# hanruihua/RDA-planner

Measured on AMD Instinct MI355X. Metric: MPC steps/sec (ADMM early stop or iter_num cap: see residuals), T=20, N_obs=200, higher is better.
Workload: dtype f64; 1 GPU; north-star: acker rectangle robot, T=20, N_obs=200 static seeded polygons, E=4, iter_num=4, iter_threshold=0.2, ro1=200; parallelism=single GPU

## Files before the change

rda_planner_amd/csrc/lammuz_device.h:

```cpp
#pragma once
#include <hip/hip_runtime.h>
#include <math.h>

#pragma clang fp contract(on)

namespace lmz {

constexpr int EMAX = 8;
constexpr int RMAX = 8;
constexpr double SIGN_TOL = 1e-12;

struct WaveLDS {
    double A[EMAX][2];
    double b[EMAX];
    double q[EMAX];
    double M[EMAX][2];
    unsigned char lamc[40];
    double vtx[28][2];
    int npv, nlv;
};
struct RobotLDS {
    double G[RMAX][2];
    double h[RMAX];
    unsigned char muc[40]; int nmv;
    double rv[28][2]; int nrv;
};

struct Sol {
    double cost; int id;
    double m, H0, H1;
    int i1, i2, j1, j2;
    double l1, l2, g1, g2;
};

struct MuCand { int k; int j0, j1; double gx, gy, eta; double P00, P01, P10, P11, det, r0, r1, rr;
                double iden;
                double idet; };

__device__ __forceinline__ void gamma_star(const MuCand &mc, double chi, double ro2, double delta,
                                           double t, double e0, double e1,
                                           double &ga0, double &ga1, double &m, double &H0, double &H1)
{
    if (mc.k == 0) { m = t; H0 = e0; H1 = e1; ga0 = 0; ga1 = 0; return; }
    if (mc.k == 1) {
        double ga = (chi * mc.eta * t - delta * mc.eta - ro2 * (mc.gx * e0 + mc.gy * e1)) * mc.iden;
        ga0 = ga; ga1 = 0; m = t - mc.eta * ga; H0 = e0 + ga * mc.gx; H1 = e1 + ga * mc.gy;
        return;
    }
    double re = mc.r0 * e0 + mc.r1 * e1;
    double beta = (delta - chi * (t + re)) * mc.iden;
    H0 = -beta * mc.r0; H1 = -beta * mc.r1;
    double d0 = H0 - e0, d1 = H1 - e1;
    ga0 = (mc.P11 * d0 - mc.P01 * d1) * mc.idet;
    ga1 = (-mc.P10 * d0 + mc.P00 * d1) * mc.idet;
    m = t + re + beta * mc.rr;
}

__device__ __forceinline__ int trs2(double q11, double q12, double q22, double c0, double c1, bool disc,
                                    double &x0, double &x1, double &x2, double &x3)
{
// ... 267 lines not shown
{
    if (lane < P.E) {
        double ax = W.A[lane][0], ay = W.A[lane][1];
        W.q[lane] = ax * P.px + ay * P.py - W.b[lane];
        W.M[lane][0] = ax * P.cs + ay * P.sn;
        W.M[lane][1] = -ax * P.sn + ay * P.cs;
    }
}

__device__ __forceinline__ void build_lists(WaveLDS &W, int E, int norm2, int lane)
{
    if (norm2) {
        if (lane == 0) { W.lamc[0] = 1; W.lamc[1] = 2; W.lamc[2] = 0; W.npv = 0; W.nlv = 3; }
    } else {
        bool vp = false; double vx = 0, vy = 0;
        if (lane < E * (E - 1) / 2) {
            int i1, i2; decode_pair(lane, E, i1, i2);
            const double a00 = W.A[i1][0], a01 = W.A[i1][1], a10 = W.A[i2][0], a11 = W.A[i2][1];
            const double det = a00 * a11 - a01 * a10;
            if (det != 0 && det * det > 1e-24 * (a00 * a00 + a01 * a01) * (a10 * a10 + a11 * a11)) {
                const double wx = W.b[i1] * a11 - a01 * W.b[i2], wy = a00 * W.b[i2] - W.b[i1] * a10, sg = det > 0 ? 1.0 : -1.0, ad = fabs(det);
                vp = true;
                for (int k = 0; k < E; ++k) {
                    const double ak0 = W.A[k][0], ak1 = W.A[k][1], bk = W.b[k];
                    const double viol = sg * (ak0 * wx + ak1 * wy - bk * det);
                    if (viol > 1e-9 * (ad + fabs(bk) * ad + fabs(ak0 * wx) + fabs(ak1 * wy))) vp = false;
                }
                vx = wx / det; vy = wy / det;
            }
        }
        const bool vs = lane < E && (W.A[lane < E ? lane : 0][0] != 0 || W.A[lane < E ? lane : 0][1] != 0);
        const unsigned long long bp = __ballot(vp), bs = __ballot(vs), below = (1ull << lane) - 1;
        const int npv = __popcll(bp), nsv = __popcll(bs);
        if (vp) { const int k = __popcll(bp & below); W.lamc[k] = (unsigned char)(1 + E + lane); W.vtx[k][0] = vx; W.vtx[k][1] = vy; }
        if (vs) W.lamc[npv + __popcll(bs & below)] = (unsigned char)(1 + lane);
        if (lane == 0) { W.lamc[npv + nsv] = 0; W.npv = npv; W.nlv = npv + nsv + 1; }
    }
}

__device__ __forceinline__ void wave_sync()
{
    __builtin_amdgcn_fence(__ATOMIC_RELEASE, "workgroup");
    __builtin_amdgcn_wave_barrier();
    __builtin_amdgcn_fence(__ATOMIC_ACQUIRE, "workgroup");
}

__device__ __forceinline__ void prepare_wave(WaveLDS &W, const Params &P, int lane)
{
    pose_products(W, P, lane);
    build_lists(W, P.E, P.norm2, lane);
    wave_sync();
}

__device__ __forceinline__ void solve_wave(WaveLDS &W, const RobotLDS &Rb, const Params &P, int lane, Sol &best)
{
    const int nm = 1 + P.R + P.R * (P.R - 1) / 2;
    const int nlv = W.nlv, nmv = Rb.nmv;
    const int half = nlv * nmv;
    best.cost = INFINITY; best.id = 0x7fffffff;
    best.m = 0; best.H0 = 0; best.H1 = 0; best.i1 = best.i2 = best.j1 = best.j2 = -1;
    best.l1 = best.l2 = best.g1 = best.g2 = 0;
    long long tprev = P.prof ? clock64() : 0;
    auto mark = [&](int k) { if (P.prof && lane == 0) { long long now = clock64(); P.prof[k] += now - tprev; tprev = now; } };
    for (int ic = 0; ic < 2; ++ic) {
        int itn = 0;
        for (int c = lane; c < half; c += 64) {
            const int ilx = c / nmv, il = W.lamc[ilx], im = Rb.muc[c - ilx * nmv];
            Sol s;
            if (eval_candidate(W, Rb, P, il, im, ic, s)) {
                s.id = 2 * (il * nm + im) + ic;
                if (s.cost < best.cost || (s.cost == best.cost && s.id < best.id)) best = s;
            }
            mark(1 + 2 * ic + (itn < 1 ? itn : 1)); ++itn;
        }
        double bc = best.cost; int bid = best.id;
#pragma unroll
        for (int off = 32; off >= 1; off >>= 1) {
            double oc = __shfl_xor(bc, off, 64); int oid = __shfl_xor(bid, off, 64);
            if (oc < bc || (oc == bc && oid < bid)) { bc = oc; bid = oid; }
        }
        unsigned long long win = __ballot(best.id == bid);
        int src = __ffsll((long long)win) - 1;
        best.cost = __shfl(best.cost, src, 64); best.id = bid;
        best.m = __shfl(best.m, src, 64); best.H0 = __shfl(best.H0, src, 64); best.H1 = __shfl(best.H1, src, 64);
        best.i1 = __shfl(best.i1, src, 64); best.i2 = __shfl(best.i2, src, 64);
        best.j1 = __shfl(best.j1, src, 64); best.j2 = __shfl(best.j2, src, 64);
        best.l1 = __shfl(best.l1, src, 64); best.l2 = __shfl(best.l2, src, 64);
        best.g1 = __shfl(best.g1, src, 64); best.g2 = __shfl(best.g2, src, 64);
        mark(5 + ic);
        if (best.m >= 0) break;
        if (ic == 0) best.cost += 0.5 * best.m * best.m;
    }
}

template <int CTRL> __device__ __forceinline__ double dpp_mov_f64(double v)
{
    int lo = __builtin_amdgcn_update_dpp(0, __double2loint(v), CTRL, 0xf, 0xf, false);
    int hi = __builtin_amdgcn_update_dpp(0, __double2hiint(v), CTRL, 0xf, 0xf, false);
    return __hiloint2double(hi, lo);
}
__device__ __forceinline__ double wave_max(double v)
{
    double o;
    o = dpp_mov_f64<0xB1>(v); v = o > v ? o : v;
    o = dpp_mov_f64<0x4E>(v); v = o > v ? o : v;
    o = dpp_mov_f64<0x141>(v); v = o > v ? o : v;
    o = dpp_mov_f64<0x140>(v); v = o > v ? o : v;
    o = __shfl_xor(v, 16, 64); v = o > v ? o : v;
    o = __shfl_xor(v, 32, 64); v = o > v ? o : v;
    return v;
}

__device__ __forceinline__ double row_max(double v)
{
    double o;
    o = dpp_mov_f64<0xB1>(v); v = o > v ? o : v;
    o = dpp_mov_f64<0x4E>(v); v = o > v ? o : v;
    o = dpp_mov_f64<0x141>(v); v = o > v ? o : v;
    o = dpp_mov_f64<0x140>(v); v = o > v ? o : v;
    return v;
}
template <int GW> struct Grp {
    static __device__ __forceinline__ unsigned long long ballot(bool p, int lane)
    {
        const unsigned long long b = __ballot(p);
        if (GW == 64) return b;
        return (b >> (lane & 48)) & 0xffffull;
    }
    static __device__ __forceinline__ double max(double v) { return GW == 64 ? wave_max(v) : row_max(v); }
    template <typename Tv> static __device__ __forceinline__ Tv bcast(Tv v, int src) { return __shfl(v, src, GW); }
};

__device__ __forceinline__ int support_neighbour(int c, int n, const unsigned char *cand, int ncand, int k)
{
    if (c == 0) { int seen = 0; for (int q = 0; q < ncand; ++q) { const int v = cand[q]; if (v >= 1 && v <= n) { if (seen == k) return v; ++seen; } } return -1; }
    if (c <= n) {
        if (k == 0) return 0;
        int seen = 1;
        for (int q = 0; q < ncand; ++q) {
            const int v = cand[q];
            if (v > n) { int a, b; decode_pair(v - 1 - n, n, a, b); if (a == c - 1 || b == c - 1) { if (seen == k) return v; ++seen; } }
        }
// ... 225 lines not shown
    if (isinf(tlo)) { chl = 0; shl = 1; } else { const double r = rsqrt(1.0 + tlo * tlo); chl = r; shl = tlo * r; }
    const double Cr = chh * chl + shh * shl, Sr = shh * chl - chh * shl;
    const double a0 = u0 * Cr - u1 * Sr, a1 = u1 * Cr + u0 * Sr;
    int i1 = -1, i2 = -1; double l1 = 0, l2 = 0;
    if (P.norm2) { i1 = 0; i2 = 1; l1 = a0; l2 = a1; }
    else {
        const double val = lane < nv ? a0 * W.vtx[lane < nv ? lane : 0][0] + a1 * W.vtx[lane < nv ? lane : 0][1] : -INFINITY, mx = Grp<GW>::max(val);
        const int kb = __ffsll((long long)Grp<GW>::ballot(val == mx, wlane)) - 1;
        decode_pair((int)W.lamc[kb] - 1 - P.E, P.E, i1, i2);
        const double a00 = W.A[i1][0], a01 = W.A[i1][1], a10 = W.A[i2][0], a11 = W.A[i2][1], det = a00 * a11 - a01 * a10;
        l1 = (a0 * a11 - a10 * a1) / det;
        l2 = (a00 * a1 - a0 * a01) / det;
        if (l1 < -1e-9 || l2 < -1e-9) return false;
        if (l1 < 0) l1 = 0;
        if (l2 < 0) l2 = 0;
    }
    const double gx = -(P.cs * a0 + P.sn * a1) - P.xi0, gy = -(-P.sn * a0 + P.cs * a1) - P.xi1;
    int j1, j2; double g1, g2;
    {
        const double val = lane < nr ? gx * Rb.rv[lane < nr ? lane : 0][0] + gy * Rb.rv[lane < nr ? lane : 0][1] : -INFINITY, mx = Grp<GW>::max(val);
        const int jb = __ffsll((long long)Grp<GW>::ballot(val == mx, wlane)) - 1;
        decode_pair((int)Rb.muc[jb] - 1 - P.R, P.R, j1, j2);
        const double a00 = Rb.G[j1][0], a01 = Rb.G[j1][1], a10 = Rb.G[j2][0], a11 = Rb.G[j2][1], det = a00 * a11 - a01 * a10;
        g1 = (gx * a11 - a10 * gy) / det;
        g2 = (a00 * gy - gx * a01) / det;
        if (g1 < -1e-9 || g2 < -1e-9) return false;
        if (g1 < 0) g1 = 0;
        if (g2 < 0) g2 = 0;
    }
    double m = P.kappa0 - g1 * Rb.h[j1] - g2 * Rb.h[j2];
    double H0 = P.xi0 + g1 * Rb.G[j1][0] + g2 * Rb.G[j2][0], H1 = P.xi1 + g1 * Rb.G[j1][1] + g2 * Rb.G[j2][1];
    if (P.norm2) {
        m += l1 * W.q[0] + l2 * W.q[1] - W.q[2];
        H0 += l1 * W.M[0][0] + l2 * W.M[1][0] - W.M[2][0]; H1 += l1 * W.M[0][1] + l2 * W.M[1][1] - W.M[2][1];
    } else {
        m += l1 * W.q[i1] + l2 * W.q[i2];
        H0 += l1 * W.M[i1][0] + l2 * W.M[i2][0]; H1 += l1 * W.M[i1][1] + l2 * W.M[i2][1];
    }
    if (m < 0) return false;
    best.i1 = i1; best.i2 = i2; best.l1 = l1; best.l2 = l2; best.j1 = j1; best.j2 = j2; best.g1 = g1; best.g2 = g2;
    best.m = m; best.H0 = H0; best.H1 = H1;
    return true;
}

__device__ __forceinline__ double lam_of(const Sol &s, int norm2, int e)
{
    if (norm2) {
        if (s.i1 < 0) return 0.0;
        return e == 0 ? s.l1 : (e == 1 ? s.l2 : (e == 2 ? -hypot(s.l1, s.l2) : 0.0));
    }
    return e == s.i1 ? s.l1 : (e == s.i2 ? s.l2 : 0.0);
}
__device__ __forceinline__ double mu_of(const Sol &s, int j) { return j == s.j1 ? s.g1 : (j == s.j2 ? s.g2 : 0.0); }

}

#pragma clang fp contract(fast)
```

rda_planner_amd/csrc/rda_hip.hip:

```cpp
#include <hip/hip_runtime.h>
#include <climits>
#include <cstdio>
#include <cstdlib>
#include <cstring>
#include <vector>
#include <chrono>
#include <memory>
#include <dlfcn.h>
#include "../../include/rda_hip.h"
#include "host_buf.h"
#include "lammuz_device.h"
#include "lammuz_cp_device.h"
#include "lammuz_ip_device.h"
#include "su_device.h"
#include "scene_device.h"
#include "lidar_device.h"
#include "track_device.h"
#include "rollout_device.h"

#define HIPCHK(x) do { hipError_t e_ = (x); if (e_ != hipSuccess) { \
    fprintf(stderr, "librda_hip: %s failed: %s (%s:%d)\n", #x, hipGetErrorString(e_), __FILE__, __LINE__); return RDA_ERR_HIP; } } while (0)

struct Ctrl {
    int stop, iters, su_status, ipm_iters, st_tmp, it_tmp;
// ... 467 lines not shown
    if (d.centre) lmz::central_normal_wave<64>(W, rb, P, lane, best);
    bad = bad || !(isfinite(best.cost) && isfinite(best.m) && isfinite(best.H0) && isfinite(best.H1));
    const int k = t * d.Nloc + nl;
    if (bad) {
        if (lane == 0) {
            store_row(d, k, failed_row(d, k));
            hint_write(d, hpar, n, t, -1);
            atomicAdd(&d.ctrl->lmz_fail, 1);
        }
        return;
    }
    const double znew = (d.c.accelerated ? 0.5 : 1.0) * (best.m > 0 ? best.m : 0.0);
    double res = 0;
    if (lane < E) {
        double v = lmz::lam_of(best, P.norm2, lane);
        res = (v - prev) * (v - prev); d.lam[o * E + lane] = v;
    } else if (lane < E + R) {
        int j = lane - E;
        double v = lmz::mu_of(best, j);
        res = (v - prev) * (v - prev); d.mu[o * R + j] = v;
    } else if (lane == E + R) {
        double old = d.z[zi];
        res = (znew - old) * (znew - old); d.z[zi] = znew;
    }
#pragma unroll
    for (int off = 32; off >= 1; off >>= 1) res += __shfl_xor(res, off, 64);
    if (lane == 0) {
        double ax = 0, ay = 0, bl = 0, mh = 0, gx = 0, gy = 0;
        for (int i = 0; i < E; ++i) {
            double v = lmz::lam_of(best, P.norm2, i);
            ax += v * W.A[i][0]; ay += v * W.A[i][1]; bl += v * W.b[i];
        }
        for (int j = 0; j < R; ++j) {
            double v = lmz::mu_of(best, j);
            mh += v * rb.h[j]; gx += v * rb.G[j][0]; gy += v * rb.G[j][1];
        }
        const double hx = gx + P.cs * ax + P.sn * ay, hy = gy - P.sn * ax + P.cs * ay;
        const double xin0 = P.xi0 + hx, xin1 = P.xi1 + hy;
        d.xi[2 * o] = xin0; d.xi[2 * o + 1] = xin1;
        const double im = ax * P.px + ay * P.py - bl - mh;
        const double zetan = zeta + im - dbar - znew;
        d.zeta[zi] = zetan;
        RowOut ro; ro.ax = ax; ro.ay = ay; ro.bl = bl; ro.c3 = mh + znew - zetan; ro.c4 = gx + xin0; ro.c5 = gy + xin1;
        ro.res = res; ro.hh = hx * hx + hy * hy;
        store_row(d, k, ro);
    }
}

__global__ __launch_bounds__(256) void k_lammuz(Dev d, int it) { lammuz_body(d, blockIdx.x, it); }

#ifdef RDA_LMZ_CLK
__device__ unsigned long long *g_lmz_clk = nullptr;
__device__ int *g_lmz_faillog = nullptr;
#endif
template <int MODE = 0, bool CW = false> __device__ __forceinline__ void lammuz_body_rows(const Dev &d, const int block, const int nblocks, const int it, const Fin &fin)
{
#pragma clang fp contract(on)
    constexpr int WPB = GS / 4;
    __shared__ lmz::WaveLDS wl[GS];
    __shared__ lmz::RobotLDS rb;
    __shared__ double rowv[MODE == 0 ? GS : 1][6];
    const int T = d.c.T, E = d.c.E, R = d.c.R;
#ifdef RDA_LMZ_CLK
    long long clk_prev = clock64(); const long long clk_in = clk_prev; bool clk_enum = false; const unsigned long long clk_wall_in = (unsigned long long)wall_clock64();
    unsigned long long *const clk_slot = g_lmz_clk ? g_lmz_clk + 16 * (size_t)(block * (GS / 4) + (threadIdx.x >> 6)) : nullptr;
#define LMZ_CLK(k) do { if (MODE == 0) { const long long now_ = clock64(); if (clk_slot && (threadIdx.x & 63) == 0) clk_slot[k] += (unsigned long long)(now_ - clk_prev); clk_prev = now_; } } while (0)
#else
#define LMZ_CLK(k) do { } while (0)
#endif
    int tb = 0, jb = 0;
    if (MODE != 2) { block_of(d, block, tb, jb); if (tb < 0) return; }
    const int lane = threadIdx.x & 63, wv = threadIdx.x >> 6, row = lane >> 4, gl = lane & 15;
    struct Early { double px, py, cs, sn, xi0, xi1, zeta, dbar, prev, vtx[4], A, b, G, h, zold; int cone, src, hpar, hint, npv, nlv; unsigned char lamc[3]; } ey;
    if (MODE == 0) {
        const int nl0 = jb * GS + wv * 4 + row, nl = nl0 < d.Nlive ? nl0 : 0, n = d.rank * d.Nloc + nl;
        ey.src = (d.slot_src && n < d.src_used) ? d.slot_src[n] : -1;
        ey.hpar = d.ctrl->hint_par & 1;
    }
    if (d.ctrl->stop) return;
    if (MODE == 2 && block * WPB >= d.ctrl->wl_count + (d.ctrl->wlc_count + 3) / 4) return;
    LMZ_CLK(0);
    if (MODE == 0) {
        const int t = tb, nl0 = jb * GS + wv * 4 + row, nl = nl0 < d.Nlive ? nl0 : 0, n = d.rank * d.Nloc + nl;
        const double *ps = d.pose + 4 * t;
        const size_t o = drow(d, n, t + 1), zi = drow(d, n, t), oc = (size_t)n * d.nt + (d.nt > 1 ? t + 1 : 0);
        ey.px = ps[0]; ey.py = ps[1]; ey.cs = ps[2]; ey.sn = ps[3];
        ey.xi0 = d.xi[2 * o]; ey.xi1 = d.xi[2 * o + 1]; ey.zeta = d.zeta[zi]; ey.dbar = d.dis[t]; ey.cone = d.cone[n];
        ey.zold = d.z[zi];
        ey.prev = *(gl < E ? &d.lam[o * E + gl] : (gl < E + R ? &d.mu[o * R + gl - E] : &d.lam[o * E]));
        {
            const size_t ao = ((size_t)n * d.nt + (d.nt > 1 ? t + 1 : 0)) * E;
            ey.A = d.A[ao * 2 + (gl < 2 * E ? gl : 0)]; ey.b = d.b[ao + (gl < E ? gl : 0)];
            ey.G = d.G[(int)threadIdx.x < 2 * R ? threadIdx.x : 0]; ey.h = d.h[(int)threadIdx.x < R ? threadIdx.x : 0];
        }
#pragma unroll
        for (int k = 0; k < 3; ++k) ey.lamc[k] = gl + 16 * k < d.oc_ls ? d.oc_lamc[oc * d.oc_ls + gl + 16 * k] : (unsigned char)0;
#pragma unroll
        for (int k = 0; k < 4; ++k) ey.vtx[k] = gl + 16 * k < d.oc_vs ? d.oc_vtx[oc * d.oc_vs + gl + 16 * k] : 0.0;
        ey.npv = d.oc_cnt[2 * oc]; ey.nlv = d.oc_cnt[2 * oc + 1];
        {
            const int key = (ey.src >= 0 && ey.src < d.src_cap) ? d.c.N + ey.src : n, tr = (it == 0 && t + 1 < T) ? t + 1 : t;
            ey.hint = d.hint[(size_t)(ey.hpar ^ 1) * d.hint_len + (size_t)tr * d.hint_stride + key];
        }
    }
    if (MODE == 0) {
        if ((int)threadIdx.x < 2 * R) rb.G[threadIdx.x >> 1][threadIdx.x & 1] = ey.G;
        if ((int)threadIdx.x < R) rb.h[threadIdx.x] = ey.h;
    } else {
        for (int i = threadIdx.x; i < 2 * R; i += 64 * WPB) rb.G[i >> 1][i & 1] = d.G[i];
        for (int i = threadIdx.x; i < R; i += 64 * WPB) rb.h[i] = d.h[i];
    }
    for (int i = threadIdx.x; i < 40; i += 64 * WPB) rb.muc[i] = d.muc[i];
    for (int i = threadIdx.x; i < 56; i += 64 * WPB) (&rb.rv[0][0])[i] = (&d.rv[0][0])[i];
    if (threadIdx.x == 0) { rb.nmv = d.nmv; rb.nrv = d.nrv; }
    const int cntP = MODE == 2 ? d.ctrl->wl_count : 1, cntC = MODE == 2 ? d.ctrl->wlc_count : 0;
    const int cnt = cntP + (cntC + 3) / 4;
    for (int base = MODE == 2 ? block * WPB : 0; base < cnt; base += MODE == 2 ? nblocks * WPB : 1) {
    if (MODE == 2) __syncthreads();
    const bool entry = MODE == 2 && base + wv < cnt;
// ... 63 lines not shown
    lmz::wave_sync();
    LMZ_CLK(2);
    const int hpar = MODE == 0 ? ey.hpar : (d.ctrl->hint_par & 1);
    const int hint_in = MODE == 0 ? ey.hint : (MODE != 2 ? hint_read(d, hpar, n, t, it == 0) : ((P.norm2 && live) ? hint_read(d, hpar, n, t, it == 0) : -1));
    bool ok = MODE != 2 && d.warm && lmz::solve_wave_warm<16>(W, rb, P, lane, hint_in, best);
    if (CW && MODE == 0 && d.warm && P.norm2 && live && !bad) ok = lmz::warm_circle<16>(W, rb, P, lane, hint_in, best);
    if (MODE == 2 && d.warm && P.norm2 && live && !bad) ok = lmz::warm_circle<16>(W, rb, P, lane, hint_in, best);
    LMZ_CLK(3);
    if (MODE != 2 && !live && !ok) {
        best.cost = 0; best.id = 0; best.m = -1; best.H0 = best.H1 = 0; best.i1 = best.i2 = best.j1 = best.j2 = -1;
        best.l1 = best.l2 = best.g1 = best.g2 = 0;
        ok = true;
    }
    unsigned long long need = __ballot(!ok);
    if (MODE == 2) {
        need = __ballot(live && !ok);
        if (!live) {
            best.cost = 0; best.id = 0; best.m = -1; best.H0 = best.H1 = 0; best.i1 = best.i2 = best.j1 = best.j2 = -1;
            best.l1 = best.l2 = best.g1 = best.g2 = 0;
        }
    }
#ifdef RDA_LMZ_STATS
    if (lane == 0) {
        const int nf = __popcll(need) >> 4;
        if (block == 0 && wv == 0) atomicAdd(&d.ctrl->lmz_stat[0], 1u);
        atomicAdd(&d.ctrl->lmz_stat[1], (unsigned)nf); atomicAdd(&d.ctrl->lmz_stat[2 + nf], 1u);
    }
#endif
    bool defer = false;
    if (MODE == 1) {
        defer = ((need >> (16 * row)) & 1) != 0 && !bad;
        if ((need >> (16 * row)) & 1) {
            best.cost = 0; best.id = 0; best.m = -1; best.H0 = best.H1 = 0; best.i1 = best.i2 = best.j1 = best.j2 = -1;
            best.l1 = best.l2 = best.g1 = best.g2 = 0;
        }
        if (defer && gl == 0 && live) {
            if (P.norm2) d.wl[d.wl_cap - 1 - atomicAdd(&d.ctrl->wlc_count, 1)] = t * GS * d.J + nl;
            else d.wl[atomicAdd(&d.ctrl->wl_count, 1)] = t * GS * d.J + nl;
        }
        need = 0;
    }
    if (MODE == 0) {
        struct Prm { int norm2; double px, py, cs, sn, xi0, xi1, kappa0; };
        __shared__ int nfail; __shared__ unsigned char flist[GS]; __shared__ Prm prm[GS]; __shared__ lmz::Sol sol[GS];
        if (threadIdx.x == 0) nfail = 0;
        __syncthreads();
        const bool mine = ((need >> (16 * row)) & 1) != 0;
        if (mine && gl == 0) {
            const int rid = wv * 4 + row; flist[atomicAdd(&nfail, 1)] = (unsigned char)rid;
            Prm &q = prm[rid]; q.norm2 = P.norm2; q.px = P.px; q.py = P.py; q.cs = P.cs; q.sn = P.sn; q.xi0 = P.xi0; q.xi1 = P.xi1; q.kappa0 = P.kappa0;
        }
        __syncthreads();
        const int nf = nfail;
        for (int i = wv; i < nf; i += WPB) {
            const int rid = flist[i];
            lmz::Params Pg;
            { const Prm &q = prm[rid]; Pg.E = E; Pg.R = R; Pg.norm2 = q.norm2; Pg.px = q.px; Pg.py = q.py; Pg.cs = q.cs; Pg.sn = q.sn; Pg.xi0 = q.xi0; Pg.xi1 = q.xi1;
              Pg.kappa0 = q.kappa0; Pg.ro2 = P.ro2; Pg.delta = P.delta; }
            lmz::Sol bg;
            lmz::solve_wave(wl[rid], rb, Pg, lane, bg);
            if (lane == 0) sol[rid] = bg;
        }
        __syncthreads();
        if (mine) best = sol[wv * 4 + row];
        need = 0;
#ifdef RDA_LMZ_CLK
        clk_enum = nf > 0;
        if (mine && gl == 0 && live && g_lmz_faillog) {
            const int k = atomicAdd(&g_lmz_faillog[0], 1);
            if (k < 200000) { g_lmz_faillog[1 + 3 * k] = hint_in; g_lmz_faillog[2 + 3 * k] = best.id >> 1; g_lmz_faillog[3 + 3 * k] = P.norm2; }
        }
#endif
    }
    LMZ_CLK(4);
    while (need) {
        const int g = (__ffsll((long long)need) - 1) >> 4;
        need &= ~(0xffffull << (16 * g));
        lmz::Params Pg;
        const int src = 16 * g;
        Pg.E = E; Pg.R = R; Pg.norm2 = __shfl(P.norm2, src, 64);
        Pg.px = __shfl(P.px, src, 64); Pg.py = __shfl(P.py, src, 64); Pg.cs = __shfl(P.cs, src, 64); Pg.sn = __shfl(P.sn, src, 64);
        Pg.xi0 = __shfl(P.xi0, src, 64); Pg.xi1 = __shfl(P.xi1, src, 64); Pg.kappa0 = __shfl(P.kappa0, src, 64);
        Pg.ro2 = P.ro2; Pg.delta = P.delta;
        lmz::Sol bg;
        lmz::solve_wave(wl[wv * 4 + g], rb, Pg, lane, bg);
        if (row == g) best = bg;
    }
    if (gl == 0 && live && !defer) hint_write(d, hpar, n, t, best.id >> 1);
    if (d.centre) lmz::central_normal_wave<16>(W, rb, P, lane, best);
    LMZ_CLK(5);
    bad = bad || !(isfinite(best.cost) && isfinite(best.m) && isfinite(best.H0) && isfinite(best.H1));
    const double znew = (d.c.accelerated ? 0.5 : 1.0) * (best.m > 0 ? best.m : 0.0);
    double res = 0;
    const bool wr = live && !bad && !defer;
    if (gl < E) {
        double v = lmz::lam_of(best, P.norm2, gl);
        res = (v - prev) * (v - prev); if (wr) d.lam[o * E + gl] = v;
    } else if (gl < E + R) {
        int j = gl - E;
        double v = lmz::mu_of(best, j);
        res = (v - prev) * (v - prev); if (wr) d.mu[o * R + j] = v;
    } else if (gl == E + R) {
        const double old = MODE == 0 ? ey.zold : d.z[zi];
        res = (znew - old) * (znew - old); if (wr) d.z[zi] = znew;
    }
#pragma unroll
    for (int off = 8; off >= 1; off >>= 1) res += __shfl_xor(res, off, 16);
    if (gl == 0) {
        const int k = t * d.Nloc + nl;
        RowOut ro;
        bool have = false;
        if (live && bad) {
            ro = failed_row(d, k); have = true;
            store_row(d, k, ro);
            hint_write(d, hpar, n, t, -1);
            atomicAdd(&d.ctrl->lmz_fail, 1);
        } else if (wr) {
            double ax = 0, ay = 0, bl = 0, mh = 0, gx = 0, gy = 0;
            for (int i = 0; i < E; ++i) {
                double v = lmz::lam_of(best, P.norm2, i);
                ax += v * W.A[i][0]; ay += v * W.A[i][1]; bl += v * W.b[i];
            }
            for (int j = 0; j < R; ++j) {
                double v = lmz::mu_of(best, j);
                mh += v * rb.h[j]; gx += v * rb.G[j][0]; gy += v * rb.G[j][1];
            }
            const double hx = gx + P.cs * ax + P.sn * ay, hy = gy - P.sn * ax + P.cs * ay;
            const double xin0 = P.xi0 + hx, xin1 = P.xi1 + hy;
            d.xi[2 * o] = xin0; d.xi[2 * o + 1] = xin1;
            const double im = ax * P.px + ay * P.py - bl - mh;
            const double zetan = zeta + im - dbar - znew;
            d.zeta[zi] = zetan;
            ro.ax = ax; ro.ay = ay; ro.bl = bl; ro.c3 = mh + znew - zetan; ro.c4 = gx + xin0; ro.c5 = gy + xin1;
            ro.res = res; ro.hh = hx * hx + hy * hy; have = true;
            store_row(d, k, ro);
        }
        if (MODE == 0) {
            double *rv = rowv[wv * 4 + row];
            if (have) row_record(rv, d, ro, px0, py0);
            else { rv[0] = rv[1] = rv[2] = rv[3] = rv[4] = rv[5] = 0.0; }
        }
    }
    LMZ_CLK(6);
    if (MODE == 0) {
        __syncthreads();
        block_partial(d, tb, jb, rowv, threadIdx.x);
        if (block == 0 && threadIdx.x == 0) d.ctrl->pose_ok = 1;
    }
    LMZ_CLK(7);
#ifdef RDA_LMZ_CLK
    if (MODE == 0 && clk_slot && (threadIdx.x & 63) == 0) {
        const unsigned long long tot = (unsigned long long)(clock64() - clk_in);
        clk_slot[8] += 1; clk_slot[9] += tot; if (tot > clk_slot[10]) clk_slot[10] = tot;
        clk_slot[13] = clk_wall_in; clk_slot[14] = (unsigned long long)wall_clock64();
        if (clk_enum) { clk_slot[11] += 1; clk_slot[12] += tot; }
    }
#endif
    }
#undef LMZ_CLK
}

__global__ __launch_bounds__(64 * GS / 4) void k_lammuz_rows(Dev d, int it, Fin fin) { warm_kernargs<sizeof(Dev) + sizeof(int) + sizeof(Fin)>(); lammuz_body_rows<0, true>(d, blockIdx.x, gridDim.x, it, fin); }
__global__ __launch_bounds__(64 * GS / 4, 2) void k_lammuz_rows_dense(Dev d, int it, Fin fin) { lammuz_body_rows<0>(d, blockIdx.x, gridDim.x, it, fin); }
__global__ __launch_bounds__(64 * GS / 4, 3) void k_lammuz_rows_fast(Dev d, int it) { lammuz_body_rows<1>(d, blockIdx.x, gridDim.x, it, Fin{}); }
__global__ __launch_bounds__(64 * GS / 4, 1) void k_lammuz_enum(Dev d, int it) { lammuz_body_rows<2>(d, blockIdx.x, gridDim.x, it, Fin{}); }

constexpr int FPB = 256 / GS;
__device__ __forceinline__ void finalize_body(const Dev &d, const int block, const int nblocks, const int it, const Fin &fin)
{
#pragma clang fp contract(on)
    __shared__ double rowv[FPB][GS][6];
    if (it >= 0 && d.ctrl->stop) return;
    const int T = d.c.T, g = threadIdx.x / GS, row = threadIdx.x % GS;
    const int B = block * FPB + g, t = B / d.J, j = B - t * d.J, nl = GS * j + row;
    double *rv = rowv[g][row];
    if (B < T * d.J && nl < d.Nlive) {
        const int k = t * d.Nloc + nl;
        RowOut ro; ro.ax = coef_arr(d, d.rank, 0)[k]; ro.ay = coef_arr(d, d.rank, 1)[k]; ro.bl = coef_arr(d, d.rank, 2)[k];
        ro.c3 = coef_arr(d, d.rank, 3)[k]; ro.c4 = coef_arr(d, d.rank, 4)[k]; ro.c5 = coef_arr(d, d.rank, 5)[k];
        ro.res = coef_arr(d, d.rank, 6)[k]; ro.hh = coef_arr(d, d.rank, 7)[k];
        row_record(rv, d, ro, d.pose[4 * t], d.pose[4 * t + 1]);
    } else { rv[0] = rv[1] = rv[2] = rv[3] = rv[4] = rv[5] = 0.0; }
    __syncthreads();
    if (B < T * d.J) block_partial(d, t, j, rowv[g], row);
    if (block == 0 && threadIdx.x == 0) d.ctrl->pose_ok = 1;
}
__global__ __launch_bounds__(256) void k_lmz_finalize(Dev d, int it, Fin fin) { finalize_body(d, blockIdx.x, gridDim.x, it, fin); }

template <int NX, int MX> __device__ __forceinline__ void lammuz_cp_body(const Dev &d, const int block)
{
    const int T = d.c.T, E = d.c.E, R = d.c.R;
    if (d.ctrl->stop) return;
    const int w = block * blockDim.x + threadIdx.x;
    if (d.obstacle_num == 0) {
        if (w < T && d.rank == (d.c.N - 1) / d.Nloc) {
            const int i = w * d.Nloc + (d.c.N - 1) % d.Nloc;
            coef_arr(d, d.rank, 0)[i] = 0; coef_arr(d, d.rank, 1)[i] = 0; coef_arr(d, d.rank, 2)[i] = 0;
            coef_arr(d, d.rank, 8)[i] = coef_arr(d, d.rank, 3)[i];
        }
        return;
    }
    if (w >= d.Nlive * T) return;
    const int nl = w % d.Nlive, t = w / d.Nlive, n = d.rank * d.Nloc + nl;
    const size_t ao = ((size_t)n * d.nt + (d.nt > 1 ? t + 1 : 0)) * E, o = drow(d, n, t + 1), zi = drow(d, n, t);
    const int k = t * d.Nloc + nl;
    double A[16], b[8];
    for (int i = 0; i < 2 * E; ++i) A[i] = d.A[ao * 2 + i];
    for (int i = 0; i < E; ++i) b[i] = d.b[ao + i];
// ... 1368 lines not shown
extern "C" int rda_upload_trace(rda_handle *H, int K, const double *nom_s, const double *nom_u, const double *ref_s, const double *ref_speed)
{
    if (!H || K < 1 || !nom_s || !nom_u || !ref_s || !ref_speed) return RDA_ERR_ARG;
    const size_t ns = traj_s(H->d.c.T), nu = traj_u(H->d.c.T);
    TraceSet t;
    if (t.alloc((size_t)K, ns, nu)) return RDA_ERR_HIP;
    HIPCHK(hipMemcpy(t.s, nom_s, K * ns * sizeof(double), hipMemcpyHostToDevice));
    HIPCHK(hipMemcpy(t.u, nom_u, K * nu * sizeof(double), hipMemcpyHostToDevice));
    HIPCHK(hipMemcpy(t.ref, ref_s, K * ns * sizeof(double), hipMemcpyHostToDevice));
    HIPCHK(hipMemcpy(t.speed, ref_speed, K * sizeof(double), hipMemcpyHostToDevice));
    H->trace = std::move(t);
    return RDA_OK;
}

extern "C" int rda_enqueue_step(rda_handle *H, int k)
{
    if (!H || k < 0 || k >= H->trace.K) return RDA_ERR_ARG;
    const size_t ns = traj_s(H->d.c.T), nu = traj_u(H->d.c.T);
    return enqueue_admm(H, H->trace.s + k * ns, H->trace.u + k * nu, H->trace.ref + k * ns, H->trace.speed + k,
                        H->trace.out_u + k * nu, H->trace.out_s + k * ns, H->trace.info + k);
}

extern "C" int rda_enqueue_range(rda_handle *H, int k0, int k1)
{
    if (!H || k0 < 0 || k1 > H->trace.K || k0 > k1) return RDA_ERR_ARG;
    for (int k = k0; k < k1; ++k) { int rc = rda_enqueue_step(H, k); if (rc != RDA_OK) return rc; }
    return RDA_OK;
}

#ifdef RDA_LMZ_CLK
extern "C" int rda_debug_lmz_clk(rda_handle *H, unsigned long long *out, int max_waves)
{
    static unsigned long long *buf = nullptr; static int cap = 0;
    static hbuf::Group &keep = *new hbuf::Group;
    HIPCHK(hipStreamSynchronize(H->stream));
    if (!buf) {
        hbuf::Group g; unsigned long long *b;
        if (g.dev(&b, (size_t)max_waves * 16)) return RDA_ERR_HIP;
        HIPCHK(hipMemcpyToSymbol(HIP_SYMBOL(g_lmz_clk), &b, sizeof(b)));
        keep.d.push_back(std::move(g.d[0])); buf = b; cap = max_waves;
        return RDA_OK;
    }
    if (max_waves < 0) {
        static int *flog = nullptr;
        if (!flog) {
            hbuf::Group g; int *f;
            if (g.dev(&f, 1 + 3 * 200000)) return RDA_ERR_HIP;
            HIPCHK(hipMemcpyToSymbol(HIP_SYMBOL(g_lmz_faillog), &f, sizeof(f)));
            keep.d.push_back(std::move(g.d[0])); flog = f;
            return RDA_OK;
        }
        HIPCHK(hipMemcpy(out, flog, (1 + 3 * 200000) * sizeof(int), hipMemcpyDeviceToHost));
        HIPCHK(hipMemset(flog, 0, sizeof(int)));
        return RDA_OK;
    }
    if (max_waves > cap) return RDA_ERR_ARG;
    HIPCHK(hipMemcpy(out, buf, (size_t)max_waves * 16 * sizeof(unsigned long long), hipMemcpyDeviceToHost));
    HIPCHK(hipMemset(buf, 0, (size_t)cap * 16 * sizeof(unsigned long long)));
    return RDA_OK;
}
#endif
#ifdef RDA_LMZ_STATS
extern "C" int rda_debug_lmz_stats(rda_handle *H, unsigned *out)
{
    HIPCHK(hipStreamSynchronize(H->stream));
    HIPCHK(hipMemcpy(out, (char *)H->d.ctrl + offsetof(Ctrl, lmz_stat), 8 * sizeof(unsigned), hipMemcpyDeviceToHost));
    return RDA_OK;
}
#endif
extern "C" int rda_sync(rda_handle *H) { if (!H) return RDA_ERR_ARG; HIPCHK(hipStreamSynchronize(H->stream)); H->tick.pending_scene = 0; return RDA_OK; }

extern "C" int rda_fetch_result(rda_handle *H, int k, double *out_u, double *out_s, rda_info *info)
{
    if (!H || k < 0 || k >= H->trace.K) return RDA_ERR_ARG;
    const size_t ns = traj_s(H->d.c.T), nu = traj_u(H->d.c.T);
    HIPCHK(hipStreamSynchronize(H->stream));
    if (out_u) HIPCHK(hipMemcpy(out_u, H->trace.out_u + k * nu, nu * sizeof(double), hipMemcpyDeviceToHost));
    if (out_s) HIPCHK(hipMemcpy(out_s, H->trace.out_s + k * ns, ns * sizeof(double), hipMemcpyDeviceToHost));
    if (info) HIPCHK(hipMemcpy(info, H->trace.info + k, sizeof(rda_info), hipMemcpyDeviceToHost));
    return RDA_OK;
}

extern "C" int rda_timing_reset(rda_handle *H, int enable)
{
    if (!H) return RDA_ERR_ARG;
    HIPCHK(hipStreamSynchronize(H->stream));
    HIPCHK(hipStreamSynchronize(H->stream2));
    H->timing = enable; H->ev_used[0] = H->ev_used[1] = H->ev_used[2] = H->ev_used[3] = 0;
    return RDA_OK;
}
extern "C" int rda_timing_read(rda_handle *H, int which, double *total_ms, int *launches)
{
    if (!H || which < 0 || which > 3) return RDA_ERR_ARG;
    HIPCHK(hipStreamSynchronize(which == 3 ? H->stream2 : H->stream));
    double tot = 0; int n = 0;
    for (size_t i = 0; i + 1 < H->ev_used[which]; i += 2) {
        float ms = 0; HIPCHK(hipEventElapsedTime(&ms, H->ev[which][i], H->ev[which][i + 1]));
        tot += ms; ++n;
    }
    if (total_ms) *total_ms = tot;
    if (launches) *launches = n;
    return RDA_OK;
}

extern "C" int rda_timing_launches(rda_handle *H, int which, double *ms_out, int cap, int *launches)
{
// ... 1779 lines not shown
```

Baseline: 4186 steps/s.

## Split odd leftover failed row's enumeration across both waves in rows kernel

When the number of rows that fail the fast path is odd, the last row's first enumeration pass is cut at the primal-vertex boundary and run by both waves at once. Each wave writes a partial best to shared memory, the owning wave merges them, and it runs the second pass only if needed. This targets load imbalance where one wave enumerates alone while the other sits idle at the barrier. In exchange it adds shared-memory traffic, a merge step, and extra profiling hooks under a debug macro.

Measured after the change: 4204 steps/s (median of 5 runs). No clear change (+0.4%).

```diff
diff --git a/rda_planner_amd/csrc/lammuz_device.h b/rda_planner_amd/csrc/lammuz_device.h
--- a/rda_planner_amd/csrc/lammuz_device.h
+++ b/rda_planner_amd/csrc/lammuz_device.h
@@ -1,11 +1,26 @@
 #pragma once
+#ifdef __HIPCC__
 #include <hip/hip_runtime.h>
+#endif
 #include <math.h>
+#ifndef LMZ_HD
+#ifdef __HIPCC__
+#define LMZ_HD __device__ __forceinline__
+#else
+#define LMZ_HD inline
+#endif
+#endif
 
 #pragma clang fp contract(on)
 
 namespace lmz {
 
+LMZ_HD bool enum_better(double cost_b, int id_b, double cost_a, int id_a)
+{
+    return cost_b < cost_a || (cost_b == cost_b && cost_b == cost_a && id_b < id_a);
+}
+
+#ifdef __HIPCC__
 constexpr int EMAX = 8;
 constexpr int RMAX = 8;
 constexpr double SIGN_TOL = 1e-12;
@@ -379,42 +394,54 @@
     wave_sync();
 }
 
-__device__ __forceinline__ void solve_wave(WaveLDS &W, const RobotLDS &Rb, const Params &P, int lane, Sol &best)
-{
-    const int nm = 1 + P.R + P.R * (P.R - 1) / 2;
-    const int nlv = W.nlv, nmv = Rb.nmv;
-    const int half = nlv * nmv;
+__device__ __forceinline__ void empty_sol(Sol &best)
+{
     best.cost = INFINITY; best.id = 0x7fffffff;
     best.m = 0; best.H0 = 0; best.H1 = 0; best.i1 = best.i2 = best.j1 = best.j2 = -1;
     best.l1 = best.l2 = best.g1 = best.g2 = 0;
+}
+
+__device__ __forceinline__ void enum_pass(WaveLDS &W, const RobotLDS &Rb, const Params &P, int lane, int ic, int c_lo, int c_hi, const Sol &seed, Sol &out)
+{
+    const int nm = 1 + P.R + P.R * (P.R - 1) / 2;
+    const int nmv = Rb.nmv;
+    Sol best = seed;
     long long tprev = P.prof ? clock64() : 0;
     auto mark = [&](int k) { if (P.prof && lane == 0) { long long now = clock64(); P.prof[k] += now - tprev; tprev = now; } };
+    int itn = 0;
+    for (int c = c_lo + lane; c < c_hi; c += 64) {
+        const int ilx = c / nmv, il = W.lamc[ilx], im = Rb.muc[c - ilx * nmv];
+        Sol s;
+        if (eval_candidate(W, Rb, P, il, im, ic, s)) {
+            s.id = 2 * (il * nm + im) + ic;
+            if (s.cost < best.cost || (s.cost == best.cost && s.id < best.id)) best = s;
+        }
+        mark(1 + 2 * ic + (itn < 1 ? itn : 1)); ++itn;
+    }
+    double bc = best.cost; int bid = best.id;
+#pragma unroll
+    for (int off = 32; off >= 1; off >>= 1) {
+        double oc = __shfl_xor(bc, off, 64); int oid = __shfl_xor(bid, off, 64);
+        if (oc < bc || (oc == bc && oid < bid)) { bc = oc; bid = oid; }
+    }
+    unsigned long long win = __ballot(best.id == bid);
+    int src = __ffsll((long long)win) - 1;
+    best.cost = __shfl(best.cost, src, 64); best.id = bid;
+    best.m = __shfl(best.m, src, 64); best.H0 = __shfl(best.H0, src, 64); best.H1 = __shfl(best.H1, src, 64);
+    best.i1 = __shfl(best.i1, src, 64); best.i2 = __shfl(best.i2, src, 64);
+    best.j1 = __shfl(best.j1, src, 64); best.j2 = __shfl(best.j2, src, 64);
+    best.l1 = __shfl(best.l1, src, 64); best.l2 = __shfl(best.l2, src, 64);
+    best.g1 = __shfl(best.g1, src, 64); best.g2 = __shfl(best.g2, src, 64);
+    mark(5 + ic);
+    out = best;
+}
+
+__device__ __forceinline__ void solve_wave(WaveLDS &W, const RobotLDS &Rb, const Params &P, int lane, Sol &best)
+{
+    const int half = W.nlv * Rb.nmv;
+    empty_sol(best);
     for (int ic = 0; ic < 2; ++ic) {
-        int itn = 0;
-        for (int c = lane; c < half; c += 64) {
-            const int ilx = c / nmv, il = W.lamc[ilx], im = Rb.muc[c - ilx * nmv];
-            Sol s;
-            if (eval_candidate(W, Rb, P, il, im, ic, s)) {
-                s.id = 2 * (il * nm + im) + ic;
-                if (s.cost < best.cost || (s.cost == best.cost && s.id < best.id)) best = s;
-            }
-            mark(1 + 2 * ic + (itn < 1 ? itn : 1)); ++itn;
-        }
-        double bc = best.cost; int bid = best.id;
-#pragma unroll
-        for (int off = 32; off >= 1; off >>= 1) {
-            double oc = __shfl_xor(bc, off, 64); int oid = __shfl_xor(bid, off, 64);
-            if (oc < bc || (oc == bc && oid < bid)) { bc = oc; bid = oid; }
-        }
-        unsigned long long win = __ballot(best.id == bid);
-        int src = __ffsll((long long)win) - 1;
-        best.cost = __shfl(best.cost, src, 64); best.id = bid;
-        best.m = __shfl(best.m, src, 64); best.H0 = __shfl(best.H0, src, 64); best.H1 = __shfl(best.H1, src, 64);
-        best.i1 = __shfl(best.i1, src, 64); best.i2 = __shfl(best.i2, src, 64);
-        best.j1 = __shfl(best.j1, src, 64); best.j2 = __shfl(best.j2, src, 64);
-        best.l1 = __shfl(best.l1, src, 64); best.l2 = __shfl(best.l2, src, 64);
-        best.g1 = __shfl(best.g1, src, 64); best.g2 = __shfl(best.g2, src, 64);
-        mark(5 + ic);
+        enum_pass(W, Rb, P, lane, ic, 0, half, best, best);
         if (best.m >= 0) break;
         if (ic == 0) best.cost += 0.5 * best.m * best.m;
     }
@@ -746,6 +773,7 @@
     return e == s.i1 ? s.l1 : (e == s.i2 ? s.l2 : 0.0);
 }
 __device__ __forceinline__ double mu_of(const Sol &s, int j) { return j == s.j1 ? s.g1 : (j == s.j2 ? s.g2 : 0.0); }
+#endif
 
 }
 
diff --git a/rda_planner_amd/csrc/rda_hip.hip b/rda_planner_amd/csrc/rda_hip.hip
--- a/rda_planner_amd/csrc/rda_hip.hip
+++ b/rda_planner_amd/csrc/rda_hip.hip
@@ -543,6 +543,8 @@
 #ifdef RDA_LMZ_CLK
 __device__ unsigned long long *g_lmz_clk = nullptr;
 __device__ int *g_lmz_faillog = nullptr;
+constexpr int LMZ_PASSLOG = 1 + 3 * 100000;
+constexpr int LMZ_WAVELOG = LMZ_PASSLOG + 1 + 4 * 50000;
 #endif
 template <int MODE = 0, bool CW = false> __device__ __forceinline__ void lammuz_body_rows(const Dev &d, const int block, const int nblocks, const int it, const Fin &fin)
 {
@@ -553,9 +555,9 @@
     __shared__ double rowv[MODE == 0 ? GS : 1][6];
     const int T = d.c.T, E = d.c.E, R = d.c.R;
 #ifdef RDA_LMZ_CLK
-    long long clk_prev = clock64(); const long long clk_in = clk_prev; bool clk_enum = false; const unsigned long long clk_wall_in = (unsigned long long)wall_clock64();
+    long long clk_prev = clock64(); const long long clk_in = clk_prev; bool clk_enum = false, clk_owner = false; unsigned clk_loc[8] = {}; const unsigned long long clk_wall_in = (unsigned long long)wall_clock64();
     unsigned long long *const clk_slot = g_lmz_clk ? g_lmz_clk + 16 * (size_t)(block * (GS / 4) + (threadIdx.x >> 6)) : nullptr;
-#define LMZ_CLK(k) do { if (MODE == 0) { const long long now_ = clock64(); if (clk_slot && (threadIdx.x & 63) == 0) clk_slot[k] += (unsigned long long)(now_ - clk_prev); clk_prev = now_; } } while (0)
+#define LMZ_CLK(k) do { if (MODE == 0) { const long long now_ = clock64(); if (clk_slot && (threadIdx.x & 63) == 0) clk_slot[k] += (unsigned long long)(now_ - clk_prev); clk_loc[k] = (unsigned)(now_ - clk_prev); clk_prev = now_; } } while (0)
 #else
 #define LMZ_CLK(k) do { } while (0)
 #endif
@@ -725,23 +727,66 @@
         }
         __syncthreads();
         const int nf = nfail;
-        for (int i = wv; i < nf; i += WPB) {
-            const int rid = flist[i];
-            lmz::Params Pg;
-            { const Prm &q = prm[rid]; Pg.E = E; Pg.R = R; Pg.norm2 = q.norm2; Pg.px = q.px; Pg.py = q.py; Pg.cs = q.cs; Pg.sn = q.sn; Pg.xi0 = q.xi0; Pg.xi1 = q.xi1;
-              Pg.kappa0 = q.kappa0; Pg.ro2 = P.ro2; Pg.delta = P.delta; }
-            lmz::Sol bg;
-            lmz::solve_wave(wl[rid], rb, Pg, lane, bg);
-            if (lane == 0) sol[rid] = bg;
+#ifdef RDA_LMZ_CLK
+        __shared__ long long eprof[WPB][8];
+        auto pass_log = [&](int kind) {
+            if (lane != 0 || !g_lmz_faillog) return;
+            const long long *e = eprof[wv];
+            const int k = atomicAdd(&g_lmz_faillog[LMZ_PASSLOG], 1);
+            if (k < 50000) { int *r = g_lmz_faillog + LMZ_PASSLOG + 1 + 4 * k; r[0] = kind; r[1] = e[6] != 0; r[2] = (int)(e[1] + e[2] + e[5]); r[3] = (int)(e[3] + e[4] + e[6]); }
+        };
+#endif
+        static_assert(WPB == 2, "the odd row's pass is cut in two");
+        __shared__ lmz::Sol part[WPB];
+        const int srow = (CW && (nf & 1)) ? flist[nf - 1] : -1;
+        auto row_params = [&](int rid, lmz::Params &Pg) {
+            const Prm &q = prm[rid]; Pg.E = E; Pg.R = R; Pg.norm2 = q.norm2; Pg.px = q.px; Pg.py = q.py; Pg.cs = q.cs; Pg.sn = q.sn; Pg.xi0 = q.xi0; Pg.xi1 = q.xi1;
+            Pg.kappa0 = q.kappa0; Pg.ro2 = P.ro2; Pg.delta = P.delta;
+        };
+        for (int i = wv; i < nf + (srow >= 0 ? 1 : 0); i += WPB) {
+            const int rid = flist[i < nf ? i : nf - 1];
+            const bool split = rid == srow;
+            lmz::Params Pg; row_params(rid, Pg);
+#ifdef RDA_LMZ_CLK
+            if (g_lmz_faillog) { if (lane == 0) for (int k = 0; k < 8; ++k) eprof[wv][k] = 0; Pg.prof = eprof[wv]; }
+#endif
+            lmz::WaveLDS &Wg = wl[rid];
+            const int cut = Wg.npv * rb.nmv, half = Wg.nlv * rb.nmv;
+            lmz::Sol bg; lmz::empty_sol(bg);
+            for (int ic = 0; ic < 2; ++ic) {
+                lmz::enum_pass(Wg, rb, Pg, lane, ic, split && wv != 0 ? cut : 0, split && wv == 0 ? cut : half, bg, bg);
+                if (split || bg.m >= 0) break;
+                if (ic == 0) bg.cost += 0.5 * bg.m * bg.m;
+            }
+            if (lane == 0) { if (split) part[wv] = bg; else sol[rid] = bg; }
+#ifdef RDA_LMZ_CLK
+            pass_log((split ? 2 + 2 * wv : 0) + (Pg.norm2 ? 1 : 0));
+#endif
         }
         __syncthreads();
-        if (mine) best = sol[wv * 4 + row];
+        if (mine && wv * 4 + row != srow) best = sol[wv * 4 + row];
+        if (srow >= 0 && wv == (srow >> 2)) {
+            lmz::Sol c0 = part[0];
+            { const lmz::Sol c1 = part[1]; if (lmz::enum_better(c1.cost, c1.id, c0.cost, c0.id)) c0 = c1; }
+            if (!(c0.m >= 0)) {
+                lmz::Params Pg; row_params(srow, Pg);
+#ifdef RDA_LMZ_CLK
+                if (g_lmz_faillog) { if (lane == 0) for (int k = 0; k < 8; ++k) eprof[wv][k] = 0; Pg.prof = eprof[wv]; }
+#endif
+                c0.cost += 0.5 * c0.m * c0.m;
+                lmz::enum_pass(wl[srow], rb, Pg, lane, 1, 0, wl[srow].nlv * rb.nmv, c0, c0);
+#ifdef RDA_LMZ_CLK
+                pass_log(6 + (Pg.norm2 ? 1 : 0));
+#endif
+            }
+            if (row == (srow & 3)) best = c0;
+        }
         need = 0;
 #ifdef RDA_LMZ_CLK
-        clk_enum = nf > 0;
+        clk_enum = nf > 0; clk_owner = __ballot(mine) != 0;
         if (mine && gl == 0 && live && g_lmz_faillog) {
             const int k = atomicAdd(&g_lmz_faillog[0], 1);
-            if (k < 200000) { g_lmz_faillog[1 + 3 * k] = hint_in; g_lmz_faillog[2 + 3 * k] = best.id >> 1; g_lmz_faillog[3 + 3 * k] = P.norm2; }
+            if (k < 100000) { g_lmz_faillog[1 + 3 * k] = hint_in; g_lmz_faillog[2 + 3 * k] = best.id >> 1; g_lmz_faillog[3 + 3 * k] = P.norm2; }
         }
 #endif
     }
@@ -827,6 +872,10 @@
         clk_slot[8] += 1; clk_slot[9] += tot; if (tot > clk_slot[10]) clk_slot[10] = tot;
         clk_slot[13] = clk_wall_in; clk_slot[14] = (unsigned long long)wall_clock64();
         if (clk_enum) { clk_slot[11] += 1; clk_slot[12] += tot; }
+        if (clk_enum && g_lmz_faillog) {
+            const int k = atomicAdd(&g_lmz_faillog[LMZ_WAVELOG], 1);
+            if (k < 9000) { int *r = g_lmz_faillog + LMZ_WAVELOG + 1 + 10 * k; r[0] = clk_owner; for (int i = 0; i < 8; ++i) r[1 + i] = (int)clk_loc[i]; r[9] = (int)tot; }
+        }
     }
 #endif
     }
@@ -2301,6 +2350,8 @@
         }
         HIPCHK(hipMemcpy(out, flog, (1 + 3 * 200000) * sizeof(int), hipMemcpyDeviceToHost));
         HIPCHK(hipMemset(flog, 0, sizeof(int)));
+        HIPCHK(hipMemset(flog + LMZ_PASSLOG, 0, sizeof(int)));
+        HIPCHK(hipMemset(flog + LMZ_WAVELOG, 0, sizeof(int)));
         return RDA_OK;
     }
     if (max_waves > cap) return RDA_ERR_ARG;
```
